# martasumyk/hyperspectral_super-resolution

Hardware: AMD Instinct MI355X
Metric: Mpixel*bands/s fused (SRF + deg-3 per-band LSQ fit + apply) (higher is better)
Workload: dtype f32

## Files before the change

### hyperspectral_super-resolution_amd/csrc/hsr_fused_dev.h

```cpp
#pragma once
#include "hsr_common.h"
#include "hsr_solve.h"
#include "hsr_sync_dev.h"
#include "hsr_tree_dev.h"

namespace hsr {

__device__ __forceinline__ double ld_agent(const double* p) { return __hip_atomic_load(p, __ATOMIC_RELAXED, __HIP_MEMORY_SCOPE_AGENT); }
__device__ __forceinline__ void st_agent(double* p, double v) { __hip_atomic_store(p, v, __ATOMIC_RELAXED, __HIP_MEMORY_SCOPE_AGENT); }
__device__ __forceinline__ void stores_done_barrier() {
  asm volatile("s_waitcnt vmcnt(0)" ::: "memory");
  __syncthreads();
}

template <int DEG, int T, class Args>
__device__ __forceinline__ void lazy_fit(const Args& a, unsigned char* smem, int t) {
  constexpr int M = moment_count(DEG);
  static_assert(T == 512, "two passes of 32 lane rows");
  int* ticket = reinterpret_cast<int*>(smem);
  __syncthreads();
  if (t == 0) *ticket = (int)(__hip_atomic_fetch_add(a.lazy_counter, 1u, __ATOMIC_RELAXED, __HIP_MEMORY_SCOPE_AGENT) - a.lazy_base);
  __syncthreads();
  const int b = *ticket;
  if (b < 0 || b >= a.nb) return;
  double (*lsum)[16] = reinterpret_cast<double (*)[16]>(smem + 64);
  double* mom = reinterpret_cast<double*>(smem + 64 + 64 * 16 * 8);
  double* work = mom + 16;
  const int stride = a.nb * M, m = t & 15;
  const double* row = a.lazy_partials + (size_t)b * M + (m < M ? m : 0);
#pragma unroll
  for (int pass = 0; pass < 2; ++pass) {
    const int l = pass * 32 + (t >> 4);
    double s = 0.0;
    for (int i0 = l; i0 < a.lazy_slots; i0 += 64 * 8) {
      double v[8];
#pragma unroll
      for (int u = 0; u < 8; ++u) {
        const int i = i0 + 64 * u;
        v[u] = (i < a.lazy_slots && m < M) ? row[(size_t)i * stride] : 0.0;
      }
#pragma unroll
      for (int u = 0; u < 8; ++u) s += v[u];
    }
    lsum[l][m] = s;
  }
  __syncthreads();
  if (t < M) {
    const double s = butterfly_tree64(&lsum[0][t], 16);
    mom[t] = s;
    if (a.lazy_ready) st_agent(a.lazy_moments + (size_t)b * M + t, s);
    else a.lazy_moments[(size_t)b * M + t] = s;
  }
  if (a.lazy_ready) {
    stores_done_barrier();
    if (t == 0) __hip_atomic_fetch_add(a.lazy_ready, 1u, __ATOMIC_RELAXED, __HIP_MEMORY_SCOPE_AGENT);
    return;
  }
  __syncthreads();
  if (a.lazy_group_T > 1) {
    const int T2 = a.lazy_group_T;
    if (a.lazy_group_index != T2 - 1) return;
    double* gm = mom + 16 + kSolveWork;
    if (t < M) {
      double acc[32];
#pragma unroll
      for (int l = 0; l < 32; ++l) {
        const double lo = l < T2 ? 0.0 + (l == T2 - 1 ? mom[t] : a.lazy_group_moments[((size_t)l * a.nb + b) * M + t]) : 0.0;
        const int h = l + 32;
        const double hi = h < T2 ? 0.0 + (h == T2 - 1 ? mom[t] : a.lazy_group_moments[((size_t)h * a.nb + b) * M + t]) : 0.0;
        acc[l] = lo + hi;
      }
#pragma unroll
      for (int off = 16; off >= 1; off >>= 1)
#pragma unroll
        for (int l = 0; l < off; ++l) acc[l] = acc[l] + acc[l + off];
      gm[t] = acc[0];
      a.lazy_group_total[(size_t)b * M + t] = acc[0];
    }
    __syncthreads();
    if (t == 0) solve_band_t<DEG, true>(gm, a.lazy_min_count, a.lazy_coeffs + (size_t)b * (DEG + 1), work);
    return;
  }
  if (t == 0) solve_band_t<DEG, true>(mom, a.lazy_min_count, a.lazy_coeffs + (size_t)b * (DEG + 1), work);
}

template <int N, int T, class Args>
__device__ __forceinline__ void apply_prephase(const Args& a, unsigned char* smem, int t) {
  constexpr int kUse = T / 12 * 12;
  constexpr int U = 4;
  if (a.apply_x == nullptr) return;
  const bool gated = a.apply_ready != nullptr;
  double* cl = reinterpret_cast<double*>(smem);
  if (gated) {
    if (t == 0) wait_word_at_least(a.apply_ready, a.apply_ready_value, a.sync_error, 2u);
    __syncthreads();
    if (t < a.nb * N) cl[t] = ld_agent(a.apply_coeffs + t);
    __syncthreads();
  }
  const int q = (int)(a.out_ps >> 2);
  const uint32_t nv = (uint32_t)(a.apply_npix * q);
  const uint32_t stride = gridDim.x * (uint32_t)kUse;
  const uint32_t i0 = blockIdx.x * (uint32_t)kUse + (uint32_t)(t < kUse ? t : 0);
  const int c0 = (int)(i0 % (uint32_t)q) * 4;
  double c[4][N];
#pragma unroll
  for (int j = 0; j < 4; ++j) {
    const int ch = c0 + j < a.nb ? c0 + j : 0;
#pragma unroll
    for (int k = 0; k < N; ++k) c[j][k] = gated ? cl[ch * N + k] : a.apply_coeffs[ch * N + k];
  }
  if (gated) __syncthreads();
  if (t >= kUse) return;
  const float4* x4 = reinterpret_cast<const float4*>(a.apply_x);
  float4* o4 = reinterpret_cast<float4*>(a.apply_out);
  for (uint32_t ib = i0; ib < nv; ib += stride * U) {
    float4 v[U];
#pragma unroll
    for (int u = 0; u < U; ++u) {
      const uint32_t i = ib + u * stride;
      if (i < nv) v[u] = ld_stream(x4 + i);
    }
#pragma unroll
    for (int u = 0; u < U; ++u) {
      const uint32_t i = ib + u * stride;
      if (i >= nv) break;
      const bool m = !a.apply_mask || a.apply_mask[i / (uint32_t)q];
      float r[4] = {v[u].x, v[u].y, v[u].z, v[u].w};
#pragma unroll
      for (int j = 0; j < 4; ++j) {
        if (c0 + j < a.nb) {
          float xv = r[j];
          if (m) {
            const double xd = (double)xv;
            double y = 0.0;
#pragma unroll
            for (int k = 0; k < N; ++k) y = __dadd_rn(__dmul_rn(y, xd), c[j][k]);
            xv = (float)y;
          }
          r[j] = a.apply_clip ? (xv < 0.0f ? 0.0f : (xv > 1.0f ? 1.0f : xv)) : xv;
        }
      }
      st_stream(o4 + i, make_float4(r[0], r[1], r[2], r[3]));
    }
  }
}

}
```

### hyperspectral_super-resolution_amd/csrc/hsr_srf.hip

```cpp
#include <hip/hip_ext.h>

#include "hsr_common.h"
#include "hsr_solve.h"
#include "hsr_sync_dev.h"
#include "hsr_fused_dev.h"
#include "hsr_tree_dev.h"

namespace hsr {

struct SrfBands {
  int32_t k0[HSR_MAX_BANDS];
  int32_t klen[HSR_MAX_BANDS];
  int32_t woff[HSR_MAX_BANDS];
  int8_t band_of[8][2];
};

constexpr int kWeightCap = 1024;

typedef hsr_batch_unit SrfUnit;
static_assert(sizeof(SrfUnit) == 64 && sizeof(hsr_batch_tile) == 64, "batch records are 64 bytes");

struct SrfFit {
  double* gpart;
  int32_t* tickets;
// ... 115 lines not shown
__device__ __forceinline__ void lds_barrier() {
  asm volatile("s_waitcnt lgkmcnt(0)\n\ts_barrier" ::: "memory");
}

__device__ __forceinline__ void stage_f32(const float* p, float* stage_wave_uniform) {
  __builtin_amdgcn_global_load_lds((gptr_t)p, (lptr_t)stage_wave_uniform, 4, 0, 0);
}
__device__ __forceinline__ void stage_u8(const uint8_t* p, uint32_t* stage_wave_uniform) {
  const uintptr_t a = reinterpret_cast<uintptr_t>(p);
  __builtin_amdgcn_global_load_lds((gptr_t)(a & ~(uintptr_t)3), (lptr_t)stage_wave_uniform, 4, 0, 0);
}
__device__ __forceinline__ uint32_t staged_u8(const uint8_t* p, const uint32_t* stage, int lane) {
  return (stage[lane] >> ((reinterpret_cast<uintptr_t>(p) & 3) * 8)) & 0xffu;
}
constexpr int kTargetStageBytesPerBand = 64 * 4;
__host__ __device__ constexpr size_t target_stage_bytes(int nb) { return (size_t)nb * kTargetStageBytesPerBand + 64 * 4; }

__device__ __forceinline__ const char* unit_record_addr(const SrfUnit* units, int64_t idx, int nunits, int lane) {
  const int64_t i = idx < nunits ? idx : (int64_t)nunits - 1;
  return reinterpret_cast<const char*>(units + i) + (lane & 15) * 4;
}
__device__ __forceinline__ SrfUnit unit_from_lds(const uint32_t* us) {
  uint32_t w[15];
#pragma unroll
  for (int i = 0; i < 15; ++i) w[i] = __builtin_amdgcn_readfirstlane(us[i]);
  SrfUnit u;
  u.cube_dev = reinterpret_cast<const void*>(((uint64_t)w[1] << 32) | w[0]);
  u.real_dev = reinterpret_cast<const float*>(((uint64_t)w[3] << 32) | w[2]);
  u.mask_dev = reinterpret_cast<const uint8_t*>(((uint64_t)w[5] << 32) | w[4]);
  u.pseudo_dev = reinterpret_cast<float*>(((uint64_t)w[7] << 32) | w[6]);
  u.part_dev = reinterpret_cast<double*>(((uint64_t)w[9] << 32) | w[8]);
  u.npix = (int64_t)(((uint64_t)w[11] << 32) | w[10]);
  u.slots = (int32_t)w[12];
  u.slot = (int32_t)w[13];
  u.ngroups = (int32_t)w[14];
  u.reserved = 0;
  return u;
}

__device__ __forceinline__ bool any_nonfinite4(const float4& v) {
  float z = v.x * 0.0f;
  z = fmaf(v.y, 0.0f, z);
  z = fmaf(v.z, 0.0f, z);
  z = fmaf(v.w, 0.0f, z);
  return z != z;
}

__host__ __device__ __forceinline__ int stage_row(int nb, int ops) { return ops > nb ? nb : ops; }

template <int T>
__device__ __forceinline__ void flush_stage(const float* ostage, float* out, int64_t pix0, int npx, int nb, int ops, int t) {
  const int n4 = (npx * ops) >> 2;
  float4* dst = reinterpret_cast<float4*>(out + pix0 * ops);
  if (ops == nb) {
    const float4* src = reinterpret_cast<const float4*>(ostage);
    for (int i = t; i < n4; i += T) st_stream(dst + i, src[i]);
    return;
  }
  const int q = ops >> 2;
  for (int i = t; i < n4; i += T) {
    const int px = q == 4 ? i >> 2 : (q == 2 ? i >> 1 : (q == 1 ? i : i / 3));
    const int c = (i - px * q) * 4;
    const float* r = ostage + px * nb + c;
    st_stream(dst + i, make_float4(c < nb ? r[0] : 0.0f, c + 1 < nb ? r[1] : 0.0f, c + 2 < nb ? r[2] : 0.0f, c + 3 < nb ? r[3] : 0.0f));
  }
}

__device__ __forceinline__ double f64_of(int hi, int lo) { return __hiloint2double(hi, lo); }

template <int D>
__device__ __forceinline__ double merge_pair(double a, double b) {
  const int alo = __double2loint(a), ahi = __double2hiint(a), blo = __double2loint(b), bhi = __double2hiint(b);
  if (D == 32) {
    const auto l = __builtin_amdgcn_permlane32_swap(alo, blo, false, false);
    const auto h = __builtin_amdgcn_permlane32_swap(ahi, bhi, false, false);
    return f64_of(h[0], l[0]) + f64_of(h[1], l[1]);
  } else if (D == 16) {
    const auto l = __builtin_amdgcn_permlane16_swap(alo, blo, false, false);
    const auto h = __builtin_amdgcn_permlane16_swap(ahi, bhi, false, false);
    return f64_of(h[0], l[0]) + f64_of(h[1], l[1]);
  } else if (D == 8) {
    const int xlo = __builtin_amdgcn_update_dpp(alo, blo, 0x128, 0xf, 0xC, false), xhi = __builtin_amdgcn_update_dpp(ahi, bhi, 0x128, 0xf, 0xC, false);
    const int ylo = __builtin_amdgcn_update_dpp(blo, alo, 0x128, 0xf, 0x3, false), yhi = __builtin_amdgcn_update_dpp(bhi, ahi, 0x128, 0xf, 0x3, false);
    return f64_of(xhi, xlo) + f64_of(yhi, ylo);
  } else {
    static_assert(D == 32 || D == 16 || D == 8 || D == 4, "merge levels");
    const int xlo = __builtin_amdgcn_update_dpp(alo, blo, 0x124, 0xf, 0xA, false), xhi = __builtin_amdgcn_update_dpp(ahi, bhi, 0x124, 0xf, 0xA, false);
    const int ylo = __builtin_amdgcn_update_dpp(blo, alo, 0x12C, 0xf, 0x5, false), yhi = __builtin_amdgcn_update_dpp(bhi, ahi, 0x12C, 0xf, 0x5, false);
    return f64_of(xhi, xlo) + f64_of(yhi, ylo);
  }
}

template <int D>
__device__ __forceinline__ double plain_level(double v) {
  const int lo = __double2loint(v), hi = __double2hiint(v);
  if (D == 32) {
    const auto l = __builtin_amdgcn_permlane32_swap(lo, lo, false, false);
    const auto h = __builtin_amdgcn_permlane32_swap(hi, hi, false, false);
    return f64_of(h[0], l[0]) + f64_of(h[1], l[1]);
  }
  static_assert(D == 32 || D == 2 || D == 1, "plain levels");
  constexpr int ctrl = D == 2 ? 0x4E : 0xB1;
  return v + f64_of(__builtin_amdgcn_update_dpp(0, hi, ctrl, 0xf, 0xf, false), __builtin_amdgcn_update_dpp(0, lo, ctrl, 0xf, 0xf, false));
}

template <int D, int NIN, int NMAX>
__device__ __forceinline__ void merge_level(double (&v)[NMAX]) {
  constexpr int NOUT = (NIN + 1) / 2;
#pragma unroll
  for (int i = 0; i < NOUT; ++i) v[i] = merge_pair<D>(v[2 * i], v[2 * i + 1 < NIN ? 2 * i + 1 : NIN - 1]);
}

template <int M, int P, bool LANE_IS_PIXEL, bool COHERENT>
__device__ __forceinline__ void flush_moments(double (&acc_m)[2][M], const bool (&bval)[2], const int (&bidx)[2],
                                              double* part, int lane) {
  constexpr int N = 2 * M;
  constexpr bool kTop32 = P == 64 && LANE_IS_PIXEL;
  constexpr int N1 = kTop32 ? (N + 1) / 2 : N, N2 = (N1 + 1) / 2, N3 = (N2 + 1) / 2, N4 = (N3 + 1) / 2;
  double v[N];
#pragma unroll
  for (int j = 0; j < 2; ++j)
#pragma unroll
    for (int m = 0; m < M; ++m) {
      v[j * M + m] = acc_m[j][m];
      acc_m[j][m] = 0.0;
    }
  if (kTop32) merge_level<32, N, N>(v);
  merge_level<16, N1, N>(v);
  merge_level<8, N2, N>(v);
  merge_level<4, N3, N>(v);
#pragma unroll
  for (int q = 0; q < N4; ++q) {
    v[q] = plain_level<1>(plain_level<2>(v[q]));
    if (!LANE_IS_PIXEL) v[q] = plain_level<32>(v[q]);
  }
  const int b2 = (lane >> 2) & 1, b3 = (lane >> 3) & 1, b4 = (lane >> 4) & 1, b5 = (lane >> 5) & 1;
  const bool canonical = (lane & 3) == 0 && (LANE_IS_PIXEL || b5 == 0);
#pragma unroll
  for (int q = 0; q < N4; ++q) {
    int i = 2 * q + b2;
    bool valid = canonical && i < N3;
    i = 2 * i + b3;
    valid = valid && i < N2;
    i = 2 * i + b4;
    valid = valid && i < N1;
    if (kTop32) {
      i = 2 * i + b5;
      valid = valid && i < N;
    }
    const bool second = i >= M;
    if (valid && (second ? bval[1] : bval[0])) {
      double* dst = part + (size_t)(second ? bidx[1] : bidx[0]) * M + (i - (second ? M : 0));
      if (COHERENT)
        __hip_atomic_store(dst, v[q], __ATOMIC_RELAXED, __HIP_MEMORY_SCOPE_AGENT);
      else
        *dst = v[q];
    }
  }
}

template <int DEG>
__device__ __forceinline__ void fused_fit(const SrfFit& f, const double* part, int S, int nb, unsigned char* lds, int t) {
  constexpr int M = moment_count(DEG);
  const int R = nb * M;
  const int grp = (int)blockIdx.x & 63;
  int* flag = reinterpret_cast<int*>(lds);
  double* mom = reinterpret_cast<double*>(lds + 64);
  double* work = mom + HSR_MAX_BANDS * M;
  stores_done_barrier();
  if (t == 0) {
    const int expect = (S - grp + 63) >> 6;
    *flag = __hip_atomic_fetch_add(f.tickets + grp, 1, __ATOMIC_RELAXED, __HIP_MEMORY_SCOPE_AGENT) == expect - 1;
  }
  __syncthreads();
  if (!*flag) return;
  if (t < R) {
    const double* row = part + t;
    double s = 0.0;
    for (int i0 = grp; i0 < S; i0 += 64 * 8) {
      double v[8];
#pragma unroll
      for (int u = 0; u < 8; ++u) {
        const int i = i0 + 64 * u;
        v[u] = i < S ? ld_agent(row + (size_t)i * R) : 0.0;
      }
#pragma unroll
      for (int u = 0; u < 8; ++u) s += v[u];
    }
    st_agent(f.gpart + (size_t)grp * R + t, s);
  }
  stores_done_barrier();
  const int ngroups = S < 64 ? S : 64;
  if (t == 0) *flag = __hip_atomic_fetch_add(f.tickets + 64, 1, __ATOMIC_RELAXED, __HIP_MEMORY_SCOPE_AGENT) == ngroups - 1;
  __syncthreads();
  if (!*flag) return;
  {
    const int lane = t & 63, wave = t >> 6;
    constexpr int RW = (HSR_MAX_BANDS * M + 7) / 8;
    double v[RW];
#pragma unroll
    for (int k = 0; k < RW; ++k) {
      const int r = wave + 8 * k;
      v[k] = (r < R && lane < ngroups) ? ld_agent(f.gpart + (size_t)lane * R + r) : 0.0;
    }
#pragma unroll
    for (int k = 0; k < RW; ++k) {
      const int r = wave + 8 * k;
      const double s = wave_sum(v[k]);
      if (lane == 0 && r < R) {
        mom[r] = s;
        f.moments[r] = s;
      }
    }
  }
  __syncthreads();
  if (t < nb) solve_band_t<DEG, true>(mom + t * M, f.min_count, f.coeffs + (size_t)t * (DEG + 1), work + t * kSolveWork);
  if (t < 65) __hip_atomic_store(f.tickets + t, 0, __ATOMIC_RELAXED, __HIP_MEMORY_SCOPE_AGENT);
}

template <int DEG, bool FAST, bool WLDS, int P, bool OUTV, bool BATCH, bool APPLY = false>
__global__ __launch_bounds__(8 * P, 4) void srf_kernel(const SrfArgs a) {
  constexpr int T = 8 * P;
  constexpr int NW = T / 64;
  extern __shared__ __attribute__((aligned(16))) unsigned char smem[];
  float* tile = reinterpret_cast<float*>(smem);
  const int B = a.B;
  const int ldsB = a.ldsB;
  uint32_t* flags = reinterpret_cast<uint32_t*>(smem + (size_t)P * ldsB * 4);
  uint32_t* ustage = flags + 64;
  const float* wl = reinterpret_cast<const float*>(flags + 64 + (BATCH ? 16 : 0));
  float* ostage = const_cast<float*>(wl) + (WLDS ? a.wtaps : 0);
  const int ops = (int)a.out_ps;
  const int osr = stage_row(a.nb, ops);
  static_assert(P == 64, "one pixel per lane: the target stage is indexed by lane");
  float* ystage = ostage + (OUTV ? P * osr : 0);
  uint32_t* mstage = reinterpret_cast<uint32_t*>(ystage + a.nb * 64);
  float* prev_out = nullptr;
  int64_t prev_pix0 = 0;
  int prev_npx = 0;

#ifdef HSR_PHASE_STAMPS
  const unsigned long long rt_begin = real_time();
#endif
  const int t = threadIdx.x;
  const int lane = t & 63;
  const int wave = __builtin_amdgcn_readfirstlane(t >> 6);
  const int pl = t % P;
  const int grp = wave;
  const int nchunk = P * B / 4;

  if constexpr (APPLY && DEG > 0) apply_prephase<DEG + 1, T>(a, smem, t);

  int bk0[kBandSlots], bkl[kBandSlots], bwo[kBandSlots], bidx[kBandSlots];
  bool bval[kBandSlots];
#pragma unroll
  for (int j = 0; j < kBandSlots; ++j) {
    const int b = a.bands.band_of[grp][j];
    bval[j] = b >= 0;
    bidx[j] = bval[j] ? b : 0;
    const int bb = bidx[j];
    bk0[j] = a.bands.k0[bb];
    bkl[j] = bval[j] ? a.bands.klen[bb] : 0;
    bwo[j] = a.bands.woff[bb];
  }

  bool constants_staged = false;
  auto stage_constants = [&]() {
    if (WLDS) {
      float* wlw = const_cast<float*>(wl);
      for (int b = 0; b < a.nb; ++b) {
        const int kl = a.bands.klen[b];
        for (int i = t; i < kl; i += T) wlw[a.bands.woff[b] + i] = a.wn[(size_t)b * B + a.bands.k0[b] + i];
      }
    }
  };

#ifdef HSR_PHASE_STAMPS
  unsigned long long stamp_acc[8] = {0, 0, 0, 0, 0, 0, 0, 0};
  unsigned long long round_t0 = rt_begin;
  int round_no = 0;
#endif
  constexpr int M = DEG > 0 ? moment_count(DEG) : 1;
  double acc_m[kBandSlots][M];
  if (DEG > 0) {
#pragma unroll
    for (int j = 0; j < kBandSlots; ++j)
#pragma unroll
      for (int m = 0; m < M; ++m) acc_m[j][m] = 0.0;
  }

  SrfUnit cu;
  if (BATCH) {
    cu = a.units[blockIdx.x];
  } else {
    cu = a.one;
    cu.slot = blockIdx.x;
    cu.part_dev = a.one.part_dev + (size_t)blockIdx.x * a.nb * M;
  }
  int64_t nidx = (int64_t)blockIdx.x + gridDim.x;
  int g = cu.slot;
  bool pend = false;
  double* pend_part = nullptr;

  for (bool more = true; more;) {
    const int64_t pix0 = (int64_t)g * P;
    const int64_t left = cu.npix - pix0;
    const int npx = left < P ? (int)left : P;
    const float* src = reinterpret_cast<const float*>(cu.cube_dev) + pix0 * B;
    const bool pvalid = pl < npx;

    float yv[kBandSlots];
    uint32_t mraw = 1u;
    auto load_targets = [&]() {
      if (DEG > 0) {
        const int64_t pc = pvalid ? pix0 + pl : cu.npix - 1;
#pragma unroll
        for (int j = 0; j < kBandSlots; ++j)
          if (bval[j]) stage_f32(cu.real_dev + bidx[j] * a.real_bs + pc * a.real_ps, ystage + bidx[j] * 64);
        if (cu.mask_dev != nullptr && wave == NW - 1) stage_u8(cu.mask_dev + pc, mstage);
      }
    };
    auto wait_targets = [&]() {
      if (DEG > 0) {
        asm volatile("s_waitcnt vmcnt(0)" ::: "memory");
#pragma unroll
        for (int j = 0; j < kBandSlots; ++j) yv[j] = bval[j] ? ystage[bidx[j] * 64 + lane] : 0.0f;
        mraw = cu.mask_dev != nullptr ? staged_u8(cu.mask_dev + (pvalid ? pix0 + pl : cu.npix - 1), mstage, lane) : 1u;
      }
    };
    auto behind_the_dma = [&]() {
      load_targets();
      if (BATCH && wave == 0 && lane < 16)
        __builtin_amdgcn_global_load_lds((gptr_t)unit_record_addr(a.units, nidx, a.nunits, lane), (lptr_t)ustage, 4, 0, 0);
      if (!constants_staged) {
        stage_constants();
        constants_staged = true;
      }
      if (OUTV) flush_stage<8 * P>(ostage, prev_out, prev_pix0, prev_npx, a.nb, ops, t);
      if (BATCH && DEG > 0 && pend) {
        flush_moments<M, P, true, !BATCH>(acc_m, bval, bidx, pend_part, lane);
        pend = false;
      }
    };

    HSR_STAMP(st0);
    if (t < P) flags[t] = 0u;

    const bool fast_group = FAST && npx == P;
    if (fast_group) {
      const char* srcb = reinterpret_cast<const char*>(src);
      for (int c0 = wave * 64; c0 < nchunk; c0 += T) {
        const int c = c0 + lane;
        if (c < nchunk)
          __builtin_amdgcn_global_load_lds((gptr_t)(srcb + (size_t)c * 16), (lptr_t)(smem + (size_t)c0 * 16),
                                           16, 0, kGldsStream);
      }
    }
    behind_the_dma();
    HSR_STAMP(st1);
    __syncthreads();
    wait_targets();
    HSR_STAMP(st2);
    if (fast_group) {
      const float4* t4 = reinterpret_cast<const float4*>(smem);
      for (int c0 = t; c0 < nchunk; c0 += T * kScanBatchF32) {
        float4 v[kScanBatchF32];
#pragma unroll
        for (int u = 0; u < kScanBatchF32; ++u) {
          const int c = c0 + u * T;
          v[u] = t4[c < nchunk ? c : nchunk - 1];
        }
        bool bad = false;
#pragma unroll
        for (int u = 0; u < kScanBatchF32; ++u) bad |= any_nonfinite4(v[u]);
        if (bad) {
#pragma unroll
          for (int u = 0; u < kScanBatchF32; ++u) {
            const int c = c0 + u * T;
            const int e = (c < nchunk ? c : nchunk - 1) * 4;
            if (!finite_f32(v[u].x)) flags[(e + 0) / B] = 1u;
            if (!finite_f32(v[u].y)) flags[(e + 1) / B] = 1u;
            if (!finite_f32(v[u].z)) flags[(e + 2) / B] = 1u;
            if (!finite_f32(v[u].w)) flags[(e + 3) / B] = 1u;
          }
        }
      }
#ifdef HSR_PHASE_STAMPS
      HSR_STAMP(st3);
      if (a.stamps) { stamp_acc[0] += st1 - st0; stamp_acc[1] += st2 - st1; stamp_acc[2] += st3 - st2; }
#endif
    } else {
      for (int pp = wave; pp < npx; pp += NW) {
        bool bad = false;
        for (int k = lane; k < B; k += 64) {
          const float v = ld_stream(src + (size_t)pp * B + k);
          bad |= !finite_f32(v);
          tile[pp * ldsB + k] = v;
        }
        if (bad) flags[pp] = 1u;
      }
    }
    __syncthreads();

    HSR_STAMP(st4);
    const bool slow = flags[pl] != 0u;
    const float* v = tile + pl * ldsB;
    float accv[kBandSlots];
#pragma unroll
    for (int j = 0; j < kBandSlots; ++j) {
      float acc = 0.0f;
      const float* vs = v + bk0[j];
      if (WLDS) {
        constexpr int CH = kTapChunk / 2;
        const float4* w4 = reinterpret_cast<const float4*>(wl + bwo[j]);
        for (int i0 = 0; i0 < bkl[j]; i0 += CH) {
          float4 ww[CH / 4];
          float xv[CH];
#pragma unroll
          for (int u = 0; u < CH / 4; ++u) ww[u] = w4[(i0 >> 2) + u];
#pragma unroll
          for (int u = 0; u < CH; ++u) xv[u] = vs[i0 + u];
#pragma unroll
          for (int u = 0; u < CH / 4; ++u) {
            acc = fmaf(ww[u].x, xv[4 * u + 0], acc);
            acc = fmaf(ww[u].y, xv[4 * u + 1], acc);
            acc = fmaf(ww[u].z, xv[4 * u + 2], acc);
            acc = fmaf(ww[u].w, xv[4 * u + 3], acc);
          }
        }
      } else {
        const float* ws = a.wn + (size_t)bidx[j] * B + bk0[j];
        for (int i = 0; i < bkl[j]; ++i) acc = fmaf(ws[i], vs[i], acc);
      }
      accv[j] = acc;
    }
    if (slow) {
#pragma unroll
      for (int j = 0; j < kBandSlots; ++j) {
        if (bval[j]) {
          const float* w = a.wn + (size_t)bidx[j] * B;
          float acc = 0.0f;
          for (int k = 0; k < B; ++k) acc = fmaf(w[k], v[k], acc);
          accv[j] = acc;
        }
      }
    }
    if constexpr (!WLDS)
      if (grp == 0 && pvalid && a.out_bs == 1 && ops > a.nb && (ops & 3) == 0 && ops <= HSR_MAX_BANDS &&
          (reinterpret_cast<uintptr_t>(cu.pseudo_dev) & 15) == 0)
        for (int c = a.nb; c < ops; ++c) st_stream(cu.pseudo_dev + (pix0 + pl) * ops + c, 0.0f);
#pragma unroll
    for (int j = 0; j < kBandSlots; ++j) {
      if (bval[j]) {
        const float acc = accv[j];
        if (OUTV) ostage[pl * osr + bidx[j]] = acc;
        else if (pvalid) st_stream(cu.pseudo_dev + bidx[j] * a.out_bs + (pix0 + pl) * a.out_ps, acc);
        if (DEG > 0) {
          const float y = yv[j];
          const bool ok = pvalid && mraw != 0u && finite_f32(acc) && finite_f32(y) && acc > a.min_x && y > a.min_y;
          if (ok) {
            const double xd = (double)acc, yd = (double)y;
            acc_m[j][0] += 1.0;
            acc_m[j][2 * DEG + 1] += yd;
            double pw = 1.0;
#pragma unroll
            for (int k = 1; k <= 2 * DEG; ++k) {
              pw *= xd;
              acc_m[j][k] += pw;
              if (k <= DEG) acc_m[j][2 * DEG + 1 + k] += pw * yd;
            }
          }
        }
      }
    }
    prev_out = cu.pseudo_dev;
    prev_pix0 = pix0;
    prev_npx = npx;
    g += cu.slots;
    if (g >= cu.ngroups) {
      pend = true;
      pend_part = cu.part_dev;
      if (BATCH && nidx < a.nunits) {
        cu = unit_from_lds(ustage);
        g = cu.slot;
        nidx += gridDim.x;
      } else {
        more = false;
      }
    }
    HSR_STAMP(st5);
    lds_barrier();
#ifdef HSR_PHASE_STAMPS
    {
      HSR_STAMP(st6);
      if (a.stamps) { stamp_acc[3] += st5 - st4; stamp_acc[4] += st6 - st5; stamp_acc[5] += st6 - st0; stamp_acc[6] += 1; }
      if (a.stamps3 && t == 0) {
        const unsigned long long now = real_time();
        if (round_no < 64) a.stamps3[(size_t)blockIdx.x * 64 + round_no] = (uint32_t)(now - round_t0);
        round_t0 = now;
        ++round_no;
      }
    }
#endif
  }
  if (OUTV) flush_stage<8 * P>(ostage, prev_out, prev_pix0, prev_npx, a.nb, ops, t);
#ifdef HSR_PHASE_STAMPS
  if (a.stamps && lane == 0)
    for (int k = 0; k < 8; ++k) a.stamps[((size_t)blockIdx.x * NW + wave) * 8 + k] = stamp_acc[k];
#endif
  if (DEG > 0 && pend) flush_moments<M, P, true, !BATCH>(acc_m, bval, bidx, pend_part, lane);
  if constexpr (DEG > 0 && !BATCH)
    if (a.fit.tickets) fused_fit<DEG>(a.fit, a.one.part_dev, a.one.slots, a.nb, smem, t);
  if constexpr (APPLY && DEG > 0)
    if (a.lazy_partials) lazy_fit<DEG, T>(a, smem, t);
#ifdef HSR_PHASE_STAMPS
  if (a.stamps2 && t == 0) {
    uint32_t xcc, hw;
    asm volatile("s_getreg_b32 %0, hwreg(HW_REG_XCC_ID)" : "=s"(xcc));
    asm volatile("s_getreg_b32 %0, hwreg(HW_REG_HW_ID)" : "=s"(hw));
    unsigned long long* o = a.stamps2 + (size_t)blockIdx.x * 4;
    o[0] = rt_begin; o[1] = real_time(); o[2] = xcc; o[3] = hw;
  }
#endif
}


template <int DEG>
__device__ __forceinline__ void moments_accumulate(double (&acc)[DEG > 0 ? moment_count(DEG) : 1], float x, float y) {
  if (DEG == 0) return;
  const double xd = (double)x, yd = (double)y;
  acc[0] += 1.0;
  acc[2 * DEG + 1] += yd;
  double pw = 1.0;
#pragma unroll
  for (int k = 1; k <= 2 * DEG; ++k) {
    pw *= xd;
    acc[k] += pw;
    if (k <= DEG) acc[2 * DEG + 1 + k] += pw * yd;
  }
}

typedef unsigned short u16x2 __attribute__((ext_vector_type(2)));
__device__ __forceinline__ void u16_nodata_sweep(const uint4* t4, int nchunk, int nsamples, int B, uint32_t nd2,
                                                 uint32_t nodata, uint32_t* fl, int t) {
  constexpr int T = 512;
  for (int c0 = t; c0 < nchunk; c0 += T * kScanBatch) {
    uint4 v[kScanBatch];
#pragma unroll
    for (int u = 0; u < kScanBatch; ++u) {
      const int c = c0 + u * T;
      v[u] = t4[c < nchunk ? c : nchunk - 1];
    }
    u16x2 mn = {(unsigned short)0xffffu, (unsigned short)0xffffu};
#pragma unroll
    for (int u = 0; u < kScanBatch; ++u) {
      const uint32_t w[4] = {v[u].x ^ nd2, v[u].y ^ nd2, v[u].z ^ nd2, v[u].w ^ nd2};
#pragma unroll
      for (int q = 0; q < 4; ++q) mn = __builtin_elementwise_min(mn, __builtin_bit_cast(u16x2, w[q]));
    }
    const bool hit = mn.x == 0 || mn.y == 0;
    if (hit) {
#pragma unroll
      for (int u = 0; u < kScanBatch; ++u) {
        const int c = c0 + u * T;
        const int e = (c < nchunk ? c : nchunk - 1) * 8;
        const uint32_t w[4] = {v[u].x, v[u].y, v[u].z, v[u].w};
#pragma unroll
        for (int q = 0; q < 4; ++q) {
          if ((w[q] & 0xffffu) == (nodata & 0xffffu) && e + 2 * q < nsamples) fl[(e + 2 * q) / B] = 1u;
          if ((w[q] >> 16) == (nodata & 0xffffu) && e + 2 * q + 1 < nsamples) fl[(e + 2 * q + 1) / B] = 1u;
        }
      }
    }
  }
}

__device__ __forceinline__ float u16_band_dot(const uint16_t* tile, int e0, const float4* w4, int klen, float scale) {
  float acc = 0.0f;
  const uint32_t sh = (uint32_t)(e0 & 1) * 2u;
  const uint32_t* d32 = reinterpret_cast<const uint32_t*>(tile) + (e0 >> 1);
  for (int i0 = 0; i0 < klen; i0 += kTapChunk) {
    float4 ww[kTapChunk / 4];
    uint32_t d[kTapChunk / 2 + 1];
#pragma unroll
    for (int u = 0; u < kTapChunk / 4; ++u) ww[u] = w4[(i0 >> 2) + u];
#pragma unroll
    for (int u = 0; u <= kTapChunk / 2; ++u) d[u] = d32[(i0 >> 1) + u];
#pragma unroll
    for (int u = 0; u < kTapChunk / 4; ++u) {
      const uint32_t ea = __builtin_amdgcn_alignbyte(d[2 * u + 1], d[2 * u], sh);
      const uint32_t eb = __builtin_amdgcn_alignbyte(d[2 * u + 2], d[2 * u + 1], sh);
      acc = fmaf(ww[u].x, (float)(ea & 0xffffu) * scale, acc);
      acc = fmaf(ww[u].y, (float)(ea >> 16) * scale, acc);
      acc = fmaf(ww[u].z, (float)(eb & 0xffffu) * scale, acc);
      acc = fmaf(ww[u].w, (float)(eb >> 16) * scale, acc);
    }
  }
  return acc;
}

typedef float f32x2 __attribute__((ext_vector_type(2)));
__device__ __forceinline__ float u16_band_dot_fast(const uint16_t* tile, int e0, const float4* w4, int klen) {
  f32x2 acc = {0.0f, 0.0f};
  const uint32_t sh = (uint32_t)(e0 & 1) * 2u;
  const uint32_t* d32 = reinterpret_cast<const uint32_t*>(tile) + (e0 >> 1);
  for (int i0 = 0; i0 < klen; i0 += kTapChunk) {
    float4 ww[kTapChunk / 4];
    uint32_t d[kTapChunk / 2 + 1];
#pragma unroll
    for (int u = 0; u < kTapChunk / 4; ++u) ww[u] = w4[(i0 >> 2) + u];
#pragma unroll
    for (int u = 0; u <= kTapChunk / 2; ++u) d[u] = d32[(i0 >> 1) + u];
#pragma unroll
    for (int u = 0; u < kTapChunk / 4; ++u) {
      const uint32_t ea = __builtin_amdgcn_alignbyte(d[2 * u + 1], d[2 * u], sh);
      const uint32_t eb = __builtin_amdgcn_alignbyte(d[2 * u + 2], d[2 * u + 1], sh);
      const f32x2 x0 = {(float)(ea & 0xffffu), (float)(ea >> 16)}, x1 = {(float)(eb & 0xffffu), (float)(eb >> 16)};
      const f32x2 w0 = {ww[u].x, ww[u].y}, w1 = {ww[u].z, ww[u].w};
      acc = __builtin_elementwise_fma(w0, x0, acc);
      acc = __builtin_elementwise_fma(w1, x1, acc);
    }
  }
  return acc.x + acc.y;
}

template <int DEG, bool FAST, bool OUTV, bool BATCH>
__global__ __launch_bounds__(512, 4) void srf_u16_kernel(const SrfArgs a) {
  constexpr int P = 64, T = 512;
  extern __shared__ __attribute__((aligned(16))) unsigned char smem[];
  uint16_t* tile = reinterpret_cast<uint16_t*>(smem);
  const int B = a.B;
  uint32_t* flags = reinterpret_cast<uint32_t*>(smem + (size_t)P * B * 2);
  uint32_t* ustage = flags + 64;
  const float* wl = reinterpret_cast<const float*>(flags + 64 + (BATCH ? 16 : 0));
  const bool wlds = a.wtaps > 0;
  float* ostage = const_cast<float*>(wl) + a.wtaps;
  const int ops = (int)a.out_ps;
  const int osr = stage_row(a.nb, ops);
  float* ystage = ostage + (OUTV ? P * osr : 0);
  uint32_t* mstage = reinterpret_cast<uint32_t*>(ystage + a.nb * 64);
  float* prev_out = nullptr;
  int64_t prev_pix0 = 0;
  int prev_npx = 0;

  const int t = threadIdx.x;
  const int lane = t & 63;
  const int wave = __builtin_amdgcn_readfirstlane(t >> 6);
  const int pl = 2 * (lane & 31) + (lane >> 5), grp = wave;
  const float scale = a.scale;
  const uint32_t nd2 = (a.nodata & 0xffffu) * 0x00010001u;
  const bool has_nodata = a.nodata <= 0xffffu;

  int bk0[kBandSlots], bkl[kBandSlots], bwo[kBandSlots], bidx[kBandSlots];
  bool bval[kBandSlots];
#pragma unroll
  for (int j = 0; j < kBandSlots; ++j) {
    const int b = a.bands.band_of[grp][j];
    bval[j] = b >= 0;
    bidx[j] = bval[j] ? b : 0;
    bk0[j] = a.bands.k0[bidx[j]];
    bkl[j] = bval[j] ? a.bands.klen[bidx[j]] : 0;
    bwo[j] = a.bands.woff[bidx[j]];
  }
  if (wlds) {
    float* wlw = const_cast<float*>(wl);
    for (int b = 0; b < a.nb; ++b) {
      const int kl = a.bands.klen[b];
      for (int i = t; i < kl; i += T) wlw[a.bands.woff[b] + i] = a.wn[(size_t)b * B + a.bands.k0[b] + i];
    }
  }

  constexpr int M = DEG > 0 ? moment_count(DEG) : 1;
  double acc_m[kBandSlots][M];
  if (DEG > 0) {
#pragma unroll
    for (int j = 0; j < kBandSlots; ++j)
#pragma unroll
      for (int m = 0; m < M; ++m) acc_m[j][m] = 0.0;
  }

  SrfUnit cu;
  if (BATCH) {
    cu = a.units[blockIdx.x];
  } else {
    cu = a.one;
    cu.slot = blockIdx.x;
    cu.part_dev = a.one.part_dev + (size_t)blockIdx.x * a.nb * M;
  }
  int64_t nidx = (int64_t)blockIdx.x + gridDim.x;
  int g = cu.slot;
  bool pend = false;
  double* pend_part = nullptr;

  for (bool more = true; more;) {
    const int64_t pix0 = (int64_t)g * P;
    const int64_t left = cu.npix - pix0;
    const int npx = left < P ? (int)left : P;
    const uint16_t* src = reinterpret_cast<const uint16_t*>(cu.cube_dev) + pix0 * B;
    const bool pvalid = pl < npx;
    const int nchunk = (npx * B + 7) >> 3;

    float yv[kBandSlots];
    uint32_t mraw = 1u;
    auto load_targets = [&]() {
      if (DEG > 0) {
        const int64_t pc = pvalid ? pix0 + pl : cu.npix - 1;
#pragma unroll
        for (int j = 0; j < kBandSlots; ++j)
          if (bval[j]) stage_f32(cu.real_dev + bidx[j] * a.real_bs + pc * a.real_ps, ystage + bidx[j] * 64);
        if (cu.mask_dev != nullptr && wave == 7) stage_u8(cu.mask_dev + pc, mstage);
      }
    };
    auto wait_targets = [&]() {
      if (DEG > 0) {
        asm volatile("s_waitcnt vmcnt(0)" ::: "memory");
#pragma unroll
        for (int j = 0; j < kBandSlots; ++j) yv[j] = bval[j] ? ystage[bidx[j] * 64 + lane] : 0.0f;
        mraw = cu.mask_dev != nullptr ? staged_u8(cu.mask_dev + (pvalid ? pix0 + pl : cu.npix - 1), mstage, lane) : 1u;
      }
    };
    auto behind_the_dma = [&]() {
      load_targets();
      if (BATCH && wave == 0 && lane < 16)
        __builtin_amdgcn_global_load_lds((gptr_t)unit_record_addr(a.units, nidx, a.nunits, lane), (lptr_t)ustage, 4, 0, 0);
      if (OUTV) flush_stage<T>(ostage, prev_out, prev_pix0, prev_npx, a.nb, ops, t);
      if (BATCH && DEG > 0 && pend) {
        flush_moments<M, P, false, !BATCH>(acc_m, bval, bidx, pend_part, lane);
        pend = false;
      }
    };

    if (t < P) flags[t] = 0u;
    const bool fast_group = FAST && npx == P;
    if (fast_group) {
      const char* srcb = reinterpret_cast<const char*>(src);
      for (int c0 = wave * 64; c0 < nchunk; c0 += T) {
        const int c = c0 + lane;
        if (c < nchunk)
          __builtin_amdgcn_global_load_lds((gptr_t)(srcb + (size_t)c * 16), (lptr_t)(smem + (size_t)c0 * 16),
                                           16, 0, kGldsStream);
      }
    }
    behind_the_dma();
    if (!fast_group) {
      const int n = npx * B;
      for (int i = t; i < nchunk * 8; i += T) tile[i] = i < n ? ld_stream(src + i) : (uint16_t)0;
    }
    __syncthreads();
    wait_targets();
    if (has_nodata) {
      u16_nodata_sweep(reinterpret_cast<const uint4*>(smem), nchunk, npx * B, B, nd2, a.nodata, flags, t);
      __syncthreads();
    }

    const bool bad = flags[pl] != 0u;
#pragma unroll
    for (int j = 0; j < kBandSlots; ++j) {
      float acc = 0.0f;
      if (wlds) {
        acc = u16_band_dot(tile, pl * B + bk0[j], reinterpret_cast<const float4*>(wl + bwo[j]), bkl[j], scale);
      } else {
        const uint16_t* vs = tile + pl * B + bk0[j];
        const float* ws = a.wn + (size_t)bidx[j] * B + bk0[j];
        for (int i = 0; i < bkl[j]; ++i) acc = fmaf(ws[i], (float)vs[i] * scale, acc);
      }
      if (bad) acc = __uint_as_float(0x7fc00000u);
      if (bval[j]) {
        if (OUTV) ostage[pl * osr + bidx[j]] = acc;
        else if (pvalid) st_stream(cu.pseudo_dev + bidx[j] * a.out_bs + (pix0 + pl) * a.out_ps, acc);
        if (DEG > 0) {
          const float y = yv[j];
          const bool ok = pvalid && mraw != 0u && finite_f32(acc) && finite_f32(y) && acc > a.min_x && y > a.min_y;
          if (ok) moments_accumulate<DEG>(acc_m[j], acc, y);
        }
      }
    }
    prev_out = cu.pseudo_dev;
    prev_pix0 = pix0;
    prev_npx = npx;
    g += cu.slots;
    if (g >= cu.ngroups) {
      pend = true;
      pend_part = cu.part_dev;
      if (BATCH && nidx < a.nunits) {
        cu = unit_from_lds(ustage);
        g = cu.slot;
        nidx += gridDim.x;
      } else {
        more = false;
      }
    }
    lds_barrier();
  }
  if (OUTV) flush_stage<T>(ostage, prev_out, prev_pix0, prev_npx, a.nb, ops, t);
  if (DEG > 0 && pend) flush_moments<M, P, false, !BATCH>(acc_m, bval, bidx, pend_part, lane);
  if constexpr (DEG > 0 && !BATCH)
    if (a.fit.tickets) fused_fit<DEG>(a.fit, a.one.part_dev, a.one.slots, a.nb, smem, t);
}

__device__ __forceinline__ void glds16_nt_asm(const void* gaddr, uint32_t lds_base) {
  asm volatile("s_mov_b32 m0, %1\n\ts_nop 0\n\tglobal_load_lds_dwordx4 %0, off nt" ::"v"(gaddr), "s"(lds_base) : "memory");
}

__device__ __forceinline__ void glds4_asm(const void* gaddr, uint32_t lds_base) {
  asm volatile("s_mov_b32 m0, %1\n\ts_nop 0\n\tglobal_load_lds_dword %0, off" ::"v"(gaddr), "s"(lds_base) : "memory");
}

constexpr int kU16PrioIssue = 3, kU16PrioDots = 1;
template <int DEG, bool OUTV, bool BATCH, bool FASTU, bool APPLY = false>
__global__ __launch_bounds__(512, 4) void srf_u16_ring_kernel(const SrfArgs a) {
  constexpr int P = 64, T = 512;
  extern __shared__ __attribute__((aligned(16))) unsigned char smem[];
  const int B = a.B;
  const int tile_bytes = P * B * 2;
  uint32_t* flags = reinterpret_cast<uint32_t*>(smem + 2 * (size_t)tile_bytes);
  uint32_t* ustage = flags + 128;
  const float* wl = reinterpret_cast<const float*>(flags + 128 + (BATCH ? 32 : 0));
// ... 789 lines not shown
```

Measured before the change: 1.431 million.

## Draw lazy-fit ticket early and double-buffer apply prephase loads

The lazy-fit ticket atomic is now issued at the start of a workgroup's last group and stashed in shared staging memory, so its latency overlaps the SRF work instead of sitting on the critical path with extra barriers. The apply prephase is restructured into a double-buffered load/store pipeline with clamped loads and prefetched mask bytes, replacing the per-element guarded loads and the mask lookup inside the compute loop. The early draw relies on mstage surviving until the end of the loop and on the last-group test being right. Gated threads beyond kUse now take part in the loop with empty ranges.

Measured after the change: 1.445 million (median of 6 runs). 1.0% higher.

```diff
diff --git a/hyperspectral_super-resolution_amd/csrc/hsr_fused_dev.h b/hyperspectral_super-resolution_amd/csrc/hsr_fused_dev.h
--- a/hyperspectral_super-resolution_amd/csrc/hsr_fused_dev.h
+++ b/hyperspectral_super-resolution_amd/csrc/hsr_fused_dev.h
@@ -13,16 +13,15 @@
   __syncthreads();
 }
 
+template <class Args>
+__device__ __forceinline__ unsigned int lazy_draw(const Args& a) {
+  return atomicInc(a.lazy_counter, 0xffffffffu);
+}
+
 template <int DEG, int T, class Args>
-__device__ __forceinline__ void lazy_fit(const Args& a, unsigned char* smem, int t) {
+__device__ __forceinline__ void lazy_fit_band(const Args& a, unsigned char* smem, int t, int b) {
   constexpr int M = moment_count(DEG);
   static_assert(T == 512, "two passes of 32 lane rows");
-  int* ticket = reinterpret_cast<int*>(smem);
-  __syncthreads();
-  if (t == 0) *ticket = (int)(__hip_atomic_fetch_add(a.lazy_counter, 1u, __ATOMIC_RELAXED, __HIP_MEMORY_SCOPE_AGENT) - a.lazy_base);
-  __syncthreads();
-  const int b = *ticket;
-  if (b < 0 || b >= a.nb) return;
   double (*lsum)[16] = reinterpret_cast<double (*)[16]>(smem + 64);
   double* mom = reinterpret_cast<double*>(smem + 64 + 64 * 16 * 8);
   double* work = mom + 16;
@@ -84,10 +83,112 @@
   if (t == 0) solve_band_t<DEG, true>(mom, a.lazy_min_count, a.lazy_coeffs + (size_t)b * (DEG + 1), work);
 }
 
+template <int DEG, int T, class Args>
+__device__ __forceinline__ void lazy_fit(const Args& a, unsigned char* smem, int t) {
+  int* ticket = reinterpret_cast<int*>(smem);
+  __syncthreads();
+  if (t == 0) *ticket = (int)(lazy_draw(a) - a.lazy_base);
+  __syncthreads();
+  const int b = *ticket;
+  if (b < 0 || b >= a.nb) return;
+  lazy_fit_band<DEG, T>(a, smem, t, b);
+}
+
+constexpr int kApplyBatch = 4;
+struct ApplyBatch {
+  float4 v[kApplyBatch];
+  uint32_t m[kApplyBatch];
+};
+__device__ __forceinline__ void apply_load_x(const float4* x4, uint32_t ib, uint32_t last, uint32_t stride, ApplyBatch& bt) {
+#pragma unroll
+  for (int u = 0; u < kApplyBatch; ++u) {
+    const uint32_t i = ib + u * stride;
+    bt.v[u] = ld_stream(x4 + (i < last ? i : last));
+  }
+}
+__device__ __forceinline__ void apply_load_m(const uint8_t* mask, uint32_t pb, uint32_t plast, uint32_t pstride, ApplyBatch& bt) {
+#pragma unroll
+  for (int u = 0; u < kApplyBatch; ++u) {
+    const uint32_t p = pb + u * pstride;
+    bt.m[u] = mask ? (uint32_t)mask[p < plast ? p : plast] : 1u;
+  }
+}
+
+template <int N, class Args>
+__device__ __forceinline__ void apply_store(const Args& a, const ApplyBatch& bt, const double (&c)[4][N], int c0, uint32_t ib,
+                                            uint32_t end, uint32_t stride) {
+  float4* o4 = reinterpret_cast<float4*>(a.apply_out);
+#pragma unroll
+  for (int u = 0; u < kApplyBatch; ++u) {
+    const uint32_t i = ib + u * stride;
+    if (i >= end) break;
+    const bool m = bt.m[u] != 0;
+    float r[4] = {bt.v[u].x, bt.v[u].y, bt.v[u].z, bt.v[u].w};
+#pragma unroll
+    for (int j = 0; j < 4; ++j) {
+      if (c0 + j < a.nb) {
+        float xv = r[j];
+        if (m) {
+          const double xd = (double)xv;
+          double y = 0.0;
+#pragma unroll
+          for (int k = 0; k < N; ++k) y = __dadd_rn(__dmul_rn(y, xd), c[j][k]);
+          xv = (float)y;
+        }
+        r[j] = a.apply_clip ? (xv < 0.0f ? 0.0f : (xv > 1.0f ? 1.0f : xv)) : xv;
+      }
+    }
+    st_stream(o4 + i, make_float4(r[0], r[1], r[2], r[3]));
+  }
+}
+
+template <int N, class Args>
+__device__ __forceinline__ void apply_range(const Args& a, const double* cl, uint32_t i0, uint32_t end, uint32_t stride) {
+  constexpr int U = kApplyBatch;
+  const uint32_t q = (uint32_t)(a.out_ps >> 2);
+  const float4* x4 = reinterpret_cast<const float4*>(a.apply_x);
+  const uint8_t* mask = a.apply_mask;
+  const uint32_t pstride = stride / q, last = end - 1, plast = last / q;
+  uint32_t pb = i0 / q;
+  ApplyBatch b0, b1;
+  apply_load_x(x4, i0, last, stride, b0);
+  const int c0 = (int)(i0 - pb * q) * 4;
+  double c[4][N];
+  if (cl) {
+#pragma unroll
+    for (int j = 0; j < 4; ++j)
+#pragma unroll
+      for (int k = 0; k < N; ++k) c[j][k] = cl[(c0 + j < a.nb ? c0 + j : 0) * N + k];
+    __syncthreads();
+  } else {
+#pragma unroll
+    for (int j = 0; j < 4; ++j)
+#pragma unroll
+      for (int k = 0; k < N; ++k) c[j][k] = a.apply_coeffs[(c0 + j < a.nb ? c0 + j : 0) * N + k];
+  }
+  apply_load_m(mask, pb, plast, pstride, b0);
+  if (i0 >= end) return;
+  uint32_t ib = i0;
+  auto request = [&](ApplyBatch& bt) {
+    pb += pstride * U;
+    apply_load_x(x4, ib + stride * U, last, stride, bt);
+    apply_load_m(mask, pb, plast, pstride, bt);
+  };
+  request(b1);
+  apply_store<N>(a, b0, c, c0, ib, end, stride);
+  for (ib += stride * U; ib < end; ib += stride * U) {
+    request(b0);
+    apply_store<N>(a, b1, c, c0, ib, end, stride);
+    ib += stride * U;
+    if (ib >= end) break;
+    request(b1);
+    apply_store<N>(a, b0, c, c0, ib, end, stride);
+  }
+}
+
 template <int N, int T, class Args>
 __device__ __forceinline__ void apply_prephase(const Args& a, unsigned char* smem, int t) {
   constexpr int kUse = T / 12 * 12;
-  constexpr int U = 4;
   if (a.apply_x == nullptr) return;
   const bool gated = a.apply_ready != nullptr;
   double* cl = reinterpret_cast<double*>(smem);
@@ -97,52 +198,11 @@
     if (t < a.nb * N) cl[t] = ld_agent(a.apply_coeffs + t);
     __syncthreads();
   }
-  const int q = (int)(a.out_ps >> 2);
-  const uint32_t nv = (uint32_t)(a.apply_npix * q);
+  const uint32_t nv = (uint32_t)(a.apply_npix * (a.out_ps >> 2));
   const uint32_t stride = gridDim.x * (uint32_t)kUse;
-  const uint32_t i0 = blockIdx.x * (uint32_t)kUse + (uint32_t)(t < kUse ? t : 0);
-  const int c0 = (int)(i0 % (uint32_t)q) * 4;
-  double c[4][N];
-#pragma unroll
-  for (int j = 0; j < 4; ++j) {
-    const int ch = c0 + j < a.nb ? c0 + j : 0;
-#pragma unroll
-    for (int k = 0; k < N; ++k) c[j][k] = gated ? cl[ch * N + k] : a.apply_coeffs[ch * N + k];
-  }
-  if (gated) __syncthreads();
-  if (t >= kUse) return;
-  const float4* x4 = reinterpret_cast<const float4*>(a.apply_x);
-  float4* o4 = reinterpret_cast<float4*>(a.apply_out);
-  for (uint32_t ib = i0; ib < nv; ib += stride * U) {
-    float4 v[U];
-#pragma unroll
-    for (int u = 0; u < U; ++u) {
-      const uint32_t i = ib + u * stride;
-      if (i < nv) v[u] = ld_stream(x4 + i);
-    }
-#pragma unroll
-    for (int u = 0; u < U; ++u) {
-      const uint32_t i = ib + u * stride;
-      if (i >= nv) break;
-      const bool m = !a.apply_mask || a.apply_mask[i / (uint32_t)q];
-      float r[4] = {v[u].x, v[u].y, v[u].z, v[u].w};
-#pragma unroll
-      for (int j = 0; j < 4; ++j) {
-        if (c0 + j < a.nb) {
-          float xv = r[j];
-          if (m) {
-            const double xd = (double)xv;
-            double y = 0.0;
-#pragma unroll
-            for (int k = 0; k < N; ++k) y = __dadd_rn(__dmul_rn(y, xd), c[j][k]);
-            xv = (float)y;
-          }
-          r[j] = a.apply_clip ? (xv < 0.0f ? 0.0f : (xv > 1.0f ? 1.0f : xv)) : xv;
-        }
-      }
-      st_stream(o4 + i, make_float4(r[0], r[1], r[2], r[3]));
-    }
-  }
-}
-
-}
+  if (t >= kUse && !gated) return;
+  const uint32_t i0 = t < kUse ? blockIdx.x * (uint32_t)kUse + (uint32_t)t : nv;
+  apply_range<N>(a, gated ? cl : nullptr, i0, nv, stride);
+}
+
+}
diff --git a/hyperspectral_super-resolution_amd/csrc/hsr_srf.hip b/hyperspectral_super-resolution_amd/csrc/hsr_srf.hip
--- a/hyperspectral_super-resolution_amd/csrc/hsr_srf.hip
+++ b/hyperspectral_super-resolution_amd/csrc/hsr_srf.hip
@@ -441,12 +441,18 @@
   bool pend = false;
   double* pend_part = nullptr;
 
+  static_assert(!(APPLY && BATCH), "one unit per workgroup: its last group is known when the group starts");
+
   for (bool more = true; more;) {
     const int64_t pix0 = (int64_t)g * P;
     const int64_t left = cu.npix - pix0;
     const int npx = left < P ? (int)left : P;
     const float* src = reinterpret_cast<const float*>(cu.cube_dev) + pix0 * B;
     const bool pvalid = pl < npx;
+    const bool draw_now = APPLY && DEG > 0 && a.lazy_partials != nullptr && g + cu.slots >= cu.ngroups;
+    unsigned int drawn = 0u;
+    if constexpr (APPLY && DEG > 0)
+      if (draw_now && t == 0) drawn = lazy_draw(a);
 
     float yv[kBandSlots];
     uint32_t mraw = 1u;
@@ -540,6 +546,8 @@
       }
     }
     __syncthreads();
+    if constexpr (APPLY && DEG > 0)
+      if (draw_now && t == 0) mstage[0] = drawn - a.lazy_base;
 
     HSR_STAMP(st4);
     const bool slow = flags[pl] != 0u;
@@ -651,7 +659,13 @@
   if constexpr (DEG > 0 && !BATCH)
     if (a.fit.tickets) fused_fit<DEG>(a.fit, a.one.part_dev, a.one.slots, a.nb, smem, t);
   if constexpr (APPLY && DEG > 0)
-    if (a.lazy_partials) lazy_fit<DEG, T>(a, smem, t);
+    if (a.lazy_partials) {
+      const int b = __builtin_amdgcn_readfirstlane((int)mstage[0]);
+      if (b >= 0 && b < a.nb) {
+        __syncthreads();
+        lazy_fit_band<DEG, T>(a, smem, t, b);
+      }
+    }
 #ifdef HSR_PHASE_STAMPS
   if (a.stamps2 && t == 0) {
     uint32_t xcc, hw;
```
